# TimD1/vcfdist

Hardware: AMD Instinct MI355X
Metric: supercluster-alignments/sec (higher is better)
Workload: dtype int32; 1 GPU; wgs_synth; superclusters_per_gpu=1000000, span_dist=lognormal(median 20, sigma 1.2) clip [4,10000]

## Files before the change

### include/vcfdist_pr.h

```cpp
#ifndef VCFDIST_PR_H_
#define VCFDIST_PR_H_

#include <stddef.h>
#include <stdint.h>

#ifdef __cplusplus
extern "C" {
#endif

#define VPR_HAPS 4
#define VPR_ALNS 4

#define VPR_PTR_VARIANT 1
#define VPR_PTR_VAR_BEG 2
#define VPR_PTR_VAR_END 4
#define VPR_PTR_INS_LOC 8

#define VPR_TYPE_SUB 1
#define VPR_TYPE_INS 2
#define VPR_TYPE_DEL 3

#define VPR_ERRTYPE_TP 0
#define VPR_ERRTYPE_FP 1
#define VPR_ERRTYPE_FN 2
// ... 50 lines not shown
    const int32_t *sc_end;
    const int64_t *var_off[VPR_HAPS];
    const int32_t *var_pos[VPR_HAPS];
    const uint8_t *var_type[VPR_HAPS];
    const float   *var_qual[VPR_HAPS];
    const int64_t *var_ref_off[VPR_HAPS];
    const int32_t *var_ref_len[VPR_HAPS];
    const int64_t *var_alt_off[VPR_HAPS];
    const int32_t *var_alt_len[VPR_HAPS];
    const uint8_t *allele_pool[VPR_HAPS];
} vpr_variants;

typedef struct vpr_config {
    int32_t device;
    float   max_qual;
    double  credit_threshold;
    double  phase_threshold;
    int64_t workspace_bytes;
    int32_t band_mode;
    int32_t flags;
} vpr_config;
#define VPR_CFG_DENSE_S16 1
#define VPR_CFG_TIE_SMALL_LOGS 2
#define VPR_CFG_GUARD_ALLOC 4
#define VPR_CFG_HAP_DEDUP 16
#define VPR_CFG_KEEP_PATHS 8

typedef struct vpr_results {
    int32_t  *aln_dist;
    uint8_t  *aln_end_plane;
    uint8_t  *aln_beg_plane;
    uint32_t *aln_status;
    int32_t  *sc_phase;
    int32_t  *orig_phase_dist;
    int32_t  *swap_phase_dist;
    uint8_t  *errtype[VPR_HAPS][2];
    int32_t  *sync_group[VPR_HAPS][2];
    float    *credit[VPR_HAPS][2];
    int32_t  *ref_ed[VPR_HAPS][2];
    int32_t  *query_ed[VPR_HAPS][2];
    float    *callq[VPR_HAPS][2];
} vpr_results;

typedef struct vpr_timing {
    double ms_total;
    double ms_prep;
    double ms_fwd;
    double ms_bwd;
    double ms_walk;
    double ms_ed;
    int64_t n_fwd_launches;
    int64_t cells_dense;
    int64_t cells_touched;
    int64_t bytes_algorithmic;
    int64_t n_band_retries;
    int64_t n_tie_replays;
    double  ms_tie;
    double  ms_wall;
    double  ms_wall_phase[6];
    double  ms_host_alloc;
    double  ms_host_blocked;
    int64_t n_alignments_computed;
    int64_t n_device_allocs, n_device_frees, n_host_allocs;
    int64_t n_lane1_seen, n_lane1_finished, n_lane1_waves_dropped;
} vpr_timing;

typedef struct vpr_launch_stat {
    int32_t kind;
    int32_t threads;
    int32_t cells_per_thread;
    int32_t n_units;
    int64_t cells;
    int64_t bytes_algorithmic;
    double  ms;
    int64_t cells_dense;
    char    kernel[32];
} vpr_launch_stat;

typedef struct vpr_handle vpr_handle;

int  vpr_create(const vpr_config *cfg, vpr_handle **out);
void vpr_destroy(vpr_handle *h);
const char *vpr_last_error(const vpr_handle *h);
const char *vpr_version(void);
int vpr_selfcheck_tie_model(int max_entries);

int vpr_run(vpr_handle *h, const vpr_batch *batch, vpr_results *res);
// ... 85 lines not shown
```

### vcfdist_amd/_abi.py

```python
import ctypes as C

import numpy as np

HAPS = 4
ALNS = 4

PTR_VARIANT, PTR_VAR_BEG, PTR_VAR_END, PTR_INS_LOC = 1, 2, 4, 8
TYPE_SUB, TYPE_INS, TYPE_DEL = 1, 2, 3
ERRTYPE_TP, ERRTYPE_FP, ERRTYPE_FN, ERRTYPE_UN = 0, 1, 2, 5
PHASE_ORIG, PHASE_SWAP, PHASE_NONE = 0, 1, 2
PLANE_QUERY, PLANE_REF = 0, 1

ST_SWAP_TIE = 1
ST_WARN_REF_ED = 2
ST_WARN_QUERY_ED = 4
ST_WARN_EXCEEDS = 8
ST_WARN_ZERO_ED = 16
ST_ERR_NO_PTR = 32
ST_ERR_UNFINISHED = 64
ST_ERR_LIMIT = 128
ST_WARN_MASK = ST_WARN_REF_ED | ST_WARN_QUERY_ED | ST_WARN_EXCEEDS | ST_WARN_ZERO_ED

P_i64 = C.POINTER(C.c_int64)
P_i32 = C.POINTER(C.c_int32)
# ... 29 lines not shown
class VprConfig(C.Structure):
    _fields_ = [
        ("device", C.c_int32), ("max_qual", C.c_float),
        ("credit_threshold", C.c_double), ("phase_threshold", C.c_double),
        ("workspace_bytes", C.c_int64), ("band_mode", C.c_int32), ("flags", C.c_int32),
    ]


class VprResults(C.Structure):
    _fields_ = [
        ("aln_dist", P_i32), ("aln_end_plane", P_u8), ("aln_beg_plane", P_u8), ("aln_status", P_u32),
        ("sc_phase", P_i32), ("orig_phase_dist", P_i32), ("swap_phase_dist", P_i32),
        ("errtype", (P_u8 * 2) * HAPS), ("sync_group", (P_i32 * 2) * HAPS),
        ("credit", (P_f32 * 2) * HAPS), ("ref_ed", (P_i32 * 2) * HAPS),
        ("query_ed", (P_i32 * 2) * HAPS), ("callq", (P_f32 * 2) * HAPS),
    ]


CFG_DENSE_S16 = 1
CFG_TIE_SMALL_LOGS = 2
CFG_GUARD_ALLOC = 4
CFG_KEEP_PATHS = 8
CFG_HAP_DEDUP = 16


class VprTiming(C.Structure):
    _fields_ = [
        ("ms_total", C.c_double), ("ms_prep", C.c_double), ("ms_fwd", C.c_double),
        ("ms_bwd", C.c_double), ("ms_walk", C.c_double), ("ms_ed", C.c_double),
        ("n_fwd_launches", C.c_int64), ("cells_dense", C.c_int64), ("cells_touched", C.c_int64),
        ("bytes_algorithmic", C.c_int64), ("n_band_retries", C.c_int64),
        ("n_tie_replays", C.c_int64), ("ms_tie", C.c_double),
        ("ms_wall", C.c_double), ("ms_wall_phase", C.c_double * 6), ("ms_host_alloc", C.c_double),
        ("ms_host_blocked", C.c_double), ("n_alignments_computed", C.c_int64), ("n_device_allocs", C.c_int64), ("n_device_frees", C.c_int64),
        ("n_host_allocs", C.c_int64), ("n_lane1_seen", C.c_int64), ("n_lane1_finished", C.c_int64), ("n_lane1_waves_dropped", C.c_int64),
    ]


class VprLaunchStat(C.Structure):
    _fields_ = [
        ("kind", C.c_int32), ("threads", C.c_int32), ("cells_per_thread", C.c_int32), ("n_units", C.c_int32),
        ("cells", C.c_int64), ("bytes_algorithmic", C.c_int64), ("ms", C.c_double),
        ("cells_dense", C.c_int64), ("kernel", C.c_char * 32),
    ]


class VprSynthParams(C.Structure):
    _fields_ = [
        ("seed", C.c_uint64), ("n_sc", C.c_int32), ("len_mode", C.c_int32),
        ("len_a", C.c_double), ("len_b", C.c_double),
        ("len_min", C.c_int32), ("len_max", C.c_int32),
        ("p_repeat", C.c_double), ("var_per_base", C.c_double), ("p_snp", C.c_double),
        ("indel_mean", C.c_double), ("p_hom", C.c_double), ("p_keep", C.c_double),
        ("p_drop", C.c_double), ("max_qual", C.c_int32), ("reserved", C.c_int32),
        ("p_sv", C.c_double), ("sv_min", C.c_int32), ("sv_max", C.c_int32),
    ]


# ... 375 lines not shown
```

### vcfdist_amd/csrc/pr_api.hip

```cpp
#include <hip/hip_runtime.h>
#include <hip/hip_ext.h>
#include <dlfcn.h>

#include <algorithm>
#include <atomic>
#include <chrono>
#include <cstdarg>
#include <cstdio>
#include <cstdlib>
#include <cstring>
#include <condition_variable>
#include <deque>
#include <functional>
#include <mutex>
#include <string>
#include <thread>
#include <tuple>
#include <unordered_map>
#include <unordered_set>
#include <vector>

#include "../../include/vcfdist_pr.h"
#include "pr_device.h"
#include "pr_plan.h"
// ... 1738 lines not shown
                                  : (its != tie_s.end() ? int64_t(its->second) + 4 + (int64_t(A.y) - A.x) + (int64_t(T.y) - T.x) : int64_t(1) << 30);
                const int64_t lo_all = -(int64_t(d.Lt) - 1);
                int64_t lo0 = lo_all, hi0 = d.Lq - 1, lo1 = lo_all, hi1 = d.Lr - 1;
                if (!tie_full) {
                    lo0 = std::max<int64_t>(lo0, int64_t(A.x) - T.y - M); hi0 = std::min<int64_t>(hi0, int64_t(A.y) - T.x + M);
                    lo1 = std::max<int64_t>(lo1, -int64_t(T.y) - M); hi1 = std::min<int64_t>(hi1, -int64_t(T.x) + M);
                    if (hi0 < lo0) hi0 = lo0;
                    if (hi1 < lo1) hi1 = lo1;
                }
                N.dlo[0] = int32_t(lo0); N.dn[0] = int32_t(hi0 - lo0 + 1);
                N.dlo[1] = int32_t(lo1); N.dn[1] = int32_t(hi1 - lo1 + 1);
            }
            N.cells = int64_t(N.dn[0] + N.dn[1]) * d.Lt + 4;
            if (N.cells >= (int64_t(1) << 32) - 2)
                return fail(h, VPR_ERR_ARG, "supercluster %d alignment %d: (Lq + Lr + 2 Lt) * Lt = %lld stamps exceed the tie replay's 32-bit cell index",
                            d.sc, d.aln, (long long)N.cells);
            N.cap = tie_full ? N.cells : std::min<int64_t>(N.cells, 3 * int64_t(d.Lq + d.Lr + d.Lt) + 4096);
            if (!tie_full && (h->cfg.flags & VPR_CFG_TIE_SMALL_LOGS)) N.cap = 32;
            N.cap = (std::max<int64_t>(2, std::min<int64_t>(N.cap, int64_t(1) << 26)) + 1) & ~int64_t(1);
            int bi = 0;
            while (bi + 1 < TIE_N_BUCKETS && int64_t(TIE_BUCKETS_HOST[bi]) < N.cap) bi++;
            N.bcap = TIE_BUCKETS_HOST[bi];
            N.w_st = (N.cells + 3) & ~int64_t(3); N.w_buf = TIE_BUF_WORDS * N.cap; N.w_bk = (TIE_BKT_WORDS * N.bcap + 8 + 3) & ~int64_t(3);
            const int64_t need = N.w_st + N.w_buf + N.w_bk;
            total += need;
            largest = std::max(largest, need);
            if (early) dec_need += it->second.mode == 2 ? 256 : it->second.n_used;
            needs.push_back(N);
        }
        if (needs.empty()) return VPR_OK;
        trace("    replay: %zu jobs sized", needs.size());
        std::stable_sort(needs.begin(), needs.end(), [](const Need &x, const Need &y) { return x.cells > y.cells; });
        if (tie_job_cur + needs.size() > h->tie_jobs_cap) return fail(h, VPR_ERR_STATE, "tie round: job buffer overflow");
        const bool must = largest * 4 + 256 > scratch_bytes;
        const int64_t room = std::max<int64_t>(h->tie_budget - h->tie_bytes, 0) / 3 * 2;
        const int64_t nb_plan = std::min<int64_t>(std::max<int64_t>(std::min<int64_t>(total * 4, h->tie_scratch_max), 2 * scratch_bytes), room);
        if (must || (total * 4 + 256 > scratch_bytes && scratch_bytes < h->tie_scratch_max && nb_plan > scratch_bytes + scratch_bytes / 2)) {
            const int64_t nb = std::max<int64_t>(nb_plan, largest * 4) + 256;
            void *q = nullptr;
            int64_t got_b = nb;
            h->soft_alloc = !must;
            hipError_t e_sc = x_malloc(h, &q, size_t(nb), SITE);
            h->soft_alloc = false;
            if (e_sc != hipSuccess && must && largest * 4 + 256 < nb) {
                (void)hipGetLastError();
                got_b = largest * 4 + 256;
// ... 21 lines not shown
                int rc_ = dev_alloc(h, &h->d_tie_dec, size_t(nc));
                if (rc_) return rc_;
                h->tie_dec_cap = nc;
                tie_dec_cur = 0;
            }
            dec = h->d_tie_dec + tie_dec_cur;
            n_dec = h->d_tie_ndec + tie_dec_slot;
            tie_patch_slot = tie_dec_slot++; tie_patch_off = tie_dec_cur; tie_patch_cap = dec_cap;
            tie_dec_cur += dec_cap;
        }
        size_t k0 = 0;
        while (k0 < needs.size()) {
            int64_t words = 0;
            size_t k1 = k0;
            TieJob *jobs = h->hp_tie_jobs + tie_job_cur;
            while (k1 < needs.size()) {
                const Need &N = needs[k1];
                const int64_t need = N.w_st + N.w_buf + N.w_bk;
                if (k1 > k0 && (words + need) * 4 > scratch_bytes) break;
                TieJob &J = jobs[k1 - k0];
                memset(&J, 0, sizeof(J));
                J.a = P.work[size_t(off) + N.k];
                J.cap = int32_t(N.cap); J.bcap = int32_t(std::min<int64_t>(N.bcap, 0x7fffffff));
                J.stamp_off = words;
                J.dlo[0] = N.dlo[0]; J.dlo[1] = N.dlo[1]; J.dn[0] = N.dn[0]; J.dn[1] = N.dn[1];
                J.buf_off = words + N.w_st;
                J.bkt_off = (words + N.w_st + N.w_buf) / 2;
                if (early) {
                    const TieEarly &E = tie_early[J.a];
                    const AlnDesc o = plan_desc(h, *E.plan, size_t(E.pos));
                    J.mode = E.mode; J.n_used = E.n_used;
                    J.old_band_w = o.band_w; J.old_pitch[0] = o.pitch[0]; J.old_pitch[1] = o.pitch[1];
                    J.old_mat_off[0] = o.mat_off[0]; J.old_mat_off[1] = o.mat_off[1]; J.old_blo_off = o.blo_off;
                    J.old_arena = E.plan->arena;
                }
                words += need;
                k1++;
            }
            const int32_t nj = int32_t(k1 - k0);
            tie_job_cur += size_t(nj);
            n_tie_jobs += nj;
            if (!tc.tie_first_seen[se]) { tc.tie_first_seen[se] = true; tc.tie_first[se] = words * 4; }
            if (words * 4 > tc.tie_clean[se]) HIPCHK(h, hipMemsetAsync(scratch, 0xff, size_t(words) * 4, ks));
            tc.tie_clean[se] = 0;
            vpr_launch_stat ts_;
            memset(&ts_, 0, sizeof(ts_));
// ... 1058 lines not shown
            for (int iter = 0; na > 0; iter++) {
                HIPCHK(h, hipMemsetAsync(h->d_tie_cnt, 0, 8, st));
                hipLaunchKernelGGL(k_collect_ties, blocks(na), dim3(256), 0, st, h->d_outs, na, h->d_tie_list, h->d_tie_cnt, h->tie_list_cap);
                int32_t n_mark = 0;
                HIPCHK(h, hipMemcpyAsync(&n_mark, h->d_tie_cnt, 4, hipMemcpyDeviceToHost, st));
                HIPCHK(h, hipMemcpyAsync(&n_jobs_pre, h->d_njobs, 4, hipMemcpyDeviceToHost, st));
                HIPCHK(h, x_sync(h, st, SITE));
                n_jobs_final = (n_mark == 0);
                if (n_mark == 0) break;
                if (iter >= 3) return fail(h, VPR_ERR_STATE, "tie pass: %d alignments still marked after %d attempts", n_mark, iter);
                const int32_t n = std::min(n_mark, h->tie_list_cap);
                std::vector<int4> lst;
                lst.resize(size_t(n));
                HIPCHK(h, hipMemcpy(lst.data(), h->d_tie_list, size_t(n) * sizeof(int4), hipMemcpyDeviceToHost));
                if (h->debug) fprintf(stderr, "[vpr] final tie pass %d: %d alignments marked\n", iter, n_mark);
                if ((rc = tie_round(h->lad[2], lst.data(), n, iter > 0, nullptr))) return rc;
                if ((rc = tie_flush(h->lad[2]))) return rc;
                HIPCHK(h, x_sync(h, h->lad[2].ls, SITE));
            }
        }
        return rc;
    }

    void debug_replays() {
        if (h->debug && tie_job_total > 0) {
            std::vector<TieJob> js;
            for (const auto &blk : tie_job_blocks) js.insert(js.end(), blk.first, blk.first + blk.second);
            std::sort(js.begin(), js.end(), [](const TieJob &x, const TieJob &y) { return x.dbg_us > y.dbg_us; });
            int64_t tot_us = 0;
            for (const TieJob &J : js) tot_us += J.dbg_us;
            size_t nf1 = 0, nf2 = 0;
            for (const TieJob &J : js) { nf1 += J.pad == 1; nf2 += J.pad == 2; }
            fprintf(stderr, "[vpr] tie replay: %zu jobs, %.1f ms summed; gave up: %zu (logs), %zu (stamp grid)\n", js.size(), tot_us / 1000.0, nf1, nf2);
            for (const TieJob &J : js)
                if (J.pad == 2 && nf2-- < 4) {
                    const AlnDesc &d = h->descs[size_t(J.a)];
                    fprintf(stderr, "[vpr]   grid too small: sc %d aln %d Lq %d Lr %d Lt %d, diagonals [%d, +%d) [%d, +%d), spans q (%d, %d) t (%d, %d)\n", d.sc, d.aln, d.Lq, d.Lr, d.Lt,
                            J.dlo[0], J.dn[0], J.dlo[1], J.dn[1], h->hp_dspan[d.qs][d.sc].x, h->hp_dspan[d.qs][d.sc].y, h->hp_dspan[d.ts][d.sc].x, h->hp_dspan[d.ts][d.sc].y);
                    fprintf(stderr, "[vpr]     first cell outside: plane %d position %d row %d (wave %d), mode %d\n", J.dbg_oob[0], J.dbg_oob[1], J.dbg_oob[2], J.dbg_oob[3], J.mode);
                }
            for (size_t k = 0; k < js.size() && k < 8; k++) {
                const AlnDesc &d = h->descs[size_t(js[k].a)];
                fprintf(stderr, "[vpr]   sc %d aln %d Lq %d Lr %d Lt %d level %d: %d us, %d waves, %d BFS steps, %d cells; mode %d, consulted %d, decided %d (last in wave %d)\n", d.sc, d.aln,
                        d.Lq, d.Lr, d.Lt, int(h->level[size_t(js[k].a)]), js[k].dbg_us, js[k].dbg_waves, js[k].dbg_steps, js[k].dbg_cells,
                        js[k].mode, js[k].n_used, js[k].dbg_nres, js[k].dbg_lastw);
                fprintf(stderr, "[vpr]     us: BFS %d, patch %d, order A %d B %d suffix %d C %d, seeding %d, setup %d\n", js[k].dbg_t[0], js[k].dbg_t[1],
                        js[k].dbg_t[2], js[k].dbg_t[3], js[k].dbg_t[4], js[k].dbg_t[5], js[k].dbg_t[6], js[k].dbg_t[7]);
                fprintf(stderr, "[vpr]     narrow steps %d: %d not in one row, %d shrinking or growing, %d not reproduced, %d look-ahead steps committing %d levels\n",
                        js[k].dbg_la[0], js[k].dbg_la[1], js[k].dbg_la[2], js[k].dbg_la[3], js[k].dbg_la[4], js[k].dbg_la[5]);
            }
        }
    }

    void debug_levels() {
        if (!h->debug || h->descs.empty()) return;
        std::vector<AlnOut> outs(h->descs.size());
        if (hipMemcpy(outs.data(), h->d_outs, outs.size() * sizeof(AlnOut), hipMemcpyDeviceToHost) != hipSuccess) return;
        static const int32_t edge[6] = {0, 4, 16, 64, 256, 1024};
        for (int lv = 0; lv <= LV_DENSE; lv++) {
            int64_t n[7] = {0, 0, 0, 0, 0, 0, 0};
            double cells[7] = {0, 0, 0, 0, 0, 0, 0};
            for (size_t a = 0; a < outs.size(); a++) {
                if (h->level[a] != lv) continue;
                const AlnDesc &d = h->descs[a];
                int b = 0;
                while (b < 6 && outs[a].s > edge[b]) b++;
                n[b]++;
                cells[b] += double(d.Lq + d.Lr) * d.Lt;
            }
            int64_t tot = 0;
// ... 141 lines not shown
        HIPCHK(h, hipStreamSynchronize(st));
        phase(5);
        lapx("done");
        HIPCHK(h, hipGetLastError());
        (void)need_err_check;
        float ms = 0;
        (void)hipEventElapsedTime(&ms, t0, t1);
        h->timing.ms_total = ms;
        h->timing.ms_fwd = h->timing.ms_bwd = h->timing.ms_walk = h->timing.ms_ed = h->timing.ms_tie = 0;
        for (auto &e : h->events) {
            float m = 0;
            (void)hipEventElapsedTime(&m, e.a, e.b);
            e.st.ms = m;
            if (e.kind == 1) h->timing.ms_fwd += m;
            else if (e.kind == 2) h->timing.ms_bwd += m;
            else if (e.kind == 3) h->timing.ms_walk += m;
            else if (e.kind == 4) h->timing.ms_ed += m;
            else if (e.kind == 6) h->timing.ms_tie += m;
        }
        h->timing.n_fwd_launches = n_fwd;
        h->timing.cells_touched = cells_touched;
        h->timing.n_band_retries = n_retry;
        h->timing.n_tie_replays = n_tie_jobs;
        h->timing.n_alignments_computed = int64_t(h->descs.size()) - h->n_aliased;
        h->timing.n_lane1_seen = h->d_d1_info ? h->hp_tie_cnt[24 + 3] : 0;
        h->timing.n_lane1_finished = h->d_d1_info ? h->hp_tie_cnt[24 + 4] : 0;
        h->timing.n_lane1_waves_dropped = h->d_d1_info ? h->hp_tie_cnt[24 + 1] : 0;
#ifdef D1_CLOCKS
        if (h->debug && h->d_d1_info) {
            int32_t ck[8];
            (void)hipMemcpy(ck, h->d_d1_info + 8, 32, hipMemcpyDeviceToHost);
            fprintf(stderr, "[vpr] k_one_lane passes, longest wave (us): %.1f %.1f %.1f %.1f; pass 1 wave-rows %d of which four slots %d; pass 3 %d / %d\n", ck[0] * 0.01, ck[1] * 0.01,
                    ck[2] * 0.01, ck[3] * 0.01, ck[4], ck[5], ck[6], ck[7]);
        }
#endif
        if (h->debug && h->d_d1_info) fprintf(stderr, "[vpr] distance-1 lane level: %d waves, %d dropped, %d left; %d seen, %d finished (pass 1 %d, pass 2 %d, end cell %d)\n",
                                              h->hp_tie_cnt[24], h->hp_tie_cnt[25], h->hp_tie_cnt[26], h->hp_tie_cnt[27], h->hp_tie_cnt[28], h->hp_tie_cnt[29], h->hp_tie_cnt[30], h->hp_tie_cnt[31]);
        h->timing.ms_wall = phase_ms[5];
        for (int k = 0; k < 6; k++) h->timing.ms_wall_phase[k] = phase_ms[k];
        h->timing.ms_host_alloc = h->hs.ms_alloc;
        h->timing.ms_host_blocked = h->hs.ms_sync;
        h->timing.n_device_allocs = h->hs.n_dev_alloc;
        h->timing.n_device_frees = h->hs.n_dev_free;
        h->timing.n_host_allocs = h->hs.n_pin_alloc;
        if (h->stall_log && phase_ms[5] > stall_dump_ms) {
            std::vector<std::tuple<float, float, const char *, int>> tl;
// ... 56 lines not shown
        phase(0);
        HIPCHK(h, hipEventCreate(&t0));
        HIPCHK(h, hipEventCreate(&t1));
        HIPCHK(h, hipEventRecord(t0, st));
        for (int k = 0; k < 2; k++) {
            LadderCtx &c = h->lad[2 + k];
            c.ls = h->tie_stream[2 * k]; c.ls2 = h->tie_stream[2 * k + 1]; c.ev2 = h->ev_tie2[k];
            c.slot0 = 2 + (2 + k) * LadderCtx::N_SLOTS;
            c.fail_base = (2 + k) * int64_t(h->descs.size()) + int64_t(h->descs.size()) / 16 + 256;
        }
        int rc = VPR_OK;
        h->resident.clear();
        h->res0_cnt = 0;
        if (h->cfg.band_mode == 0) {
            if ((rc = run_dense(h->plan0, h->plan0.d_work, st, false))) return rc;
            if (!h->plan0.chunks.empty()) {
                const Chunk &c = h->plan0.chunks.back();
                h->res0_off = c.work_off; h->res0_cnt = c.count;
            }
        } else if ((rc = round0_windowed())) {
            return rc;
        }
        if ((rc = final_tie_pass())) return rc;
        debug_replays();
        debug_levels();
        lapx("final tie pass done");
        phase(3);
        if ((rc = deferred_edit_distances())) return rc;
        return finish();
    }
};

}

extern "C" {

int vpr_execute(vpr_handle *h) {
    if (!h) return VPR_ERR_ARG;
    if (!h->uploaded) return fail(h, VPR_ERR_STATE, "vpr_execute before vpr_upload");
    dist_free(h);
    for (auto &b : h->exec_blks) b.used = false;
    for (auto &b : h->exec_pins) b.used = false;
    h->hs = vpr_handle::HostStat();
    Exec x(h);
    const int rc = x.run();
    if (x.t0) (void)hipEventDestroy(x.t0);
// ... 9 lines not shown
```

### vcfdist_amd/csrc/pr_tie.hip

```cpp
#ifndef PR_TIE_HIP_
#define PR_TIE_HIP_

#define TIE_NEVER 0xffffffffu
#define TIE_N_BUCKETS 26
#define TIE_BUCKET_LIST {13u, 29u, 59u, 127u, 257u, 541u, 1109u, 2357u, 5087u, 10273u, 20753u, 42043u, 85229u, 172933u, \
                         351061u, 712697u, 1447153u, 2938679u, 5967347u, 12117689u, 24607243u, 49969847u, 101473717u,    \
                         206062531u, 418451333u, 849749479u}
__constant__ uint32_t TIE_BUCKETS[TIE_N_BUCKETS] = TIE_BUCKET_LIST;
static const uint32_t TIE_BUCKETS_HOST[TIE_N_BUCKETS] = TIE_BUCKET_LIST;

struct TieJob {
    int32_t a;
    int32_t cap;
    int32_t bcap;
    int32_t pad;
    int64_t stamp_off;
    int64_t buf_off;
    int64_t bkt_off;
    int32_t mode, n_used;
    int32_t dlo[2], dn[2];
    int32_t old_band_w, old_pitch[2], pad2;
    int64_t old_mat_off[2], old_blo_off;
    uint8_t *old_arena;
    int32_t dbg_us, dbg_steps, dbg_cells, dbg_waves, dbg_nres, dbg_lastw;
    int32_t dbg_oob[4];
    int32_t dbg_la[6];
    int32_t dbg_t[8];
};
#define TIE_BUF_WORDS 10
#define TIE_BLIST 8
#define TIE_BKT_WORDS (2 + 1 + TIE_BLIST)

__device__ __forceinline__ uint32_t tie_ld(const uint32_t *p) {
    return __hip_atomic_load(const_cast<uint32_t *>(p), __ATOMIC_RELAXED, __HIP_MEMORY_SCOPE_AGENT);
}
__device__ __forceinline__ void tie_wait() { asm volatile("s_waitcnt vmcnt(0)" ::: "memory"); }

__device__ __forceinline__ uint8_t *tie_flag_ptr(const AlnDesc &d, uint8_t *ws, const int32_t *blo_all, int p, int x, int t) {
    if (d.band_w == 16) {
        const int2 o = reinterpret_cast<const int2 *>(blo_all + d.blo_off)[t >> 2];
        const int col = x - (p ? o.y : o.x);
        if (col < 0 || col >= 16) return nullptr;
        return ws + d.mat_off[0] + size_t(t >> 2) * 128 + p * 64 + col * 4 + (t & 3);
    }
    if (d.band_w > 0) {
        const int col = x - blo_all[d.blo_off + int64_t(p) * d.Lt + t];
        if (col < 0 || col >= d.band_w) return nullptr;
        return ws + d.mat_off[p] + size_t(t) * d.pitch[p] + col;
    }
    return ws + d.mat_off[p] + size_t(t) * d.pitch[p] + x;
}

#define TIE_U 4
#define TIE_LA 4

template <int TIE_NW>
__global__ void __launch_bounds__(64 * TIE_NW) k_tie_replay(DevBatch B, const AlnDesc *__restrict__ descs,
                                                   TieJob *__restrict__ jobs, int n_jobs, uint8_t *ws,
                                                   const int32_t *__restrict__ blo_all, AlnOut *__restrict__ outs,
                                                   uint32_t *scratch, int32_t *__restrict__ n_overflow,
                                                   int4 *__restrict__ dec, int32_t *__restrict__ n_dec, int dec_cap) {
    constexpr int NT_ = 64 * TIE_NW;
    __shared__ uint32_t mmask[2][1024];
    __shared__ int lds_ntie, lds_nres;
    __shared__ int lds_cnt[3 * TIE_U][TIE_NW];
    __shared__ int lds_or[2][TIE_NW];
    __shared__ int lds_state[2][6];
    __shared__ uint32_t lds_tot[TIE_NW];
    const int j = blockIdx.x;
    if (j >= n_jobs) return;
    __builtin_amdgcn_s_setprio(3);
    const TieJob J = jobs[j];
    const int a = J.a;
    const AlnDesc d = descs[a];
    const int tid = threadIdx.x;
    const int lane = tid & 63, wv = tid >> 6;
    const unsigned long long lt_mask = (1ull << lane) - 1ull;
    int or_par = 0, st_par = 0;
    auto wg_any = [&](bool x) -> bool {
        const bool w_any = __any(x);
        if (lane == 0) lds_or[or_par][wv] = w_any ? 1 : 0;
        __syncthreads();
        bool r = false;
#pragma unroll
        for (int k = 0; k < TIE_NW; k++) r = r || lds_or[or_par][k];
        or_par ^= 1;
        return r;
    };
    const int Lq = d.Lq, Lr = d.Lr, Lt = d.Lt;
    const int s_fin = outs[a].s;
    const unsigned long long clk0 = wall_clock64();
    int dbg_steps = 0, dbg_cells = 0, dbg_waves = 0, dbg_lastw = -1, dbg_nres0 = 0;
    int dbg_la[6] = {0, 0, 0, 0, 0, 0};
    unsigned long long dbg_t[8] = {0, 0, 0, 0, 0, 0, 0, 0}, tk = clk0;
    auto lap = [&](int k) { const unsigned long long now = wall_clock64(); dbg_t[k] += now - tk; tk = now; };
    const uint8_t *seq0 = B.hap_seq[d.qs] + d.q_off, *seq1 = B.ref_seq + d.r_off;
    const int32_t *ptr0 = B.hap_ptr[d.qs] + d.q_off, *ptr1 = B.ref_ptr[d.qs] + d.r_off;
    const uint8_t *flg0 = B.hap_flag[d.qs] + d.q_off, *flg1 = B.ref_flag[d.qs] + d.r_off;
    const uint8_t *Ts = B.hap_seq[d.ts] + d.t_off, *Tf = B.hap_flag[d.ts] + d.t_off;
    const int4 *cand0 = B.cand_q[d.qs] + d.q_off, *cand1 = B.cand_r[d.qs] + d.r_off;
    const int4 *cand20 = B.cand2_q[d.qs] + d.q_off, *cand21 = B.cand2_r[d.qs] + d.r_off;

    uint32_t *stamp = scratch + J.stamp_off;
    uint32_t *buf = scratch + J.buf_off;
    const int cap = J.cap;
    uint2 *qc = reinterpret_cast<uint2 *>(buf), *qn = reinterpret_cast<uint2 *>(buf + 2 * size_t(cap));
    uint32_t *oc = buf + 4 * size_t(cap), *on = buf + 5 * size_t(cap);
    uint32_t *Fa = buf + 6 * size_t(cap), *Ha = buf + 7 * size_t(cap), *Ka = buf + 8 * size_t(cap);
    uint2 *Ta = reinterpret_cast<uint2 *>(buf + 9 * size_t(cap));
    const int tcap = cap / 2;
    unsigned long long *bfirst = reinterpret_cast<unsigned long long *>(scratch) + J.bkt_off;
    uint32_t *bcount = reinterpret_cast<uint32_t *>(bfirst + J.bcap);
    uint32_t *blist = reinterpret_cast<uint32_t *>((reinterpret_cast<uintptr_t>(bcount + J.bcap) + 15) & ~uintptr_t(15));
    const uint32_t sbase1 = uint32_t(J.dn[0]) * uint32_t(Lt);
    const uint32_t s_dummy = sbase1 + uint32_t(J.dn[1]) * uint32_t(Lt);
    bool oob = false;
    int oob_p = 0, oob_q = 0, oob_t = 0;
// ... 318 lines not shown
                    const uint32_t st = tie_ld(stamp + sidx(1 - p, srcs[k], t - 1));
                    if (st == TIE_NEVER || st < wave_lo) continue;
                    nsrc++;
                    if (best < 0 || st > best_st) { best = k; best_st = st; }
                }
                if (best < 0 || (J.mode == 2 && nsrc < 2)) continue;
                if (J.mode) {
                    const int k = atomicAdd(n_dec, 1);
                    if (k < dec_cap) dec[k] = make_int4(a, int(z.x), t, best);
                    atomicAdd(&lds_nres, 1);
                } else {
                    *fp = uint8_t((f & ~uint32_t(F_CHOICE_MASK | F_TIE)) | f_choice_bits(best));
                }
            }
            if (wg_any(oob)) { fail = true; break; }
            if (lds_nres != dbg_nres0) { dbg_nres0 = lds_nres; dbg_lastw = w; }
            if (J.mode == 1 && lds_nres >= J.n_used) { dbg_cells += n_cur; dbg_waves++; break; }
        }
        dbg_cells += n_cur; dbg_waves++;
        lap(1);
        if (w >= s_fin) break;

        const int n = n_cur;
        int done = 0;
        bool have_lam = false;
        while (true) {
            const int room = int(n_bkt) - done;
            const int take = min(room, n - done);
            const int m = done + take;
            tag++;
            const unsigned long long tagw = (unsigned long long)(~tag) << 32;
            for (int b0 = tid; b0 < int(n_bkt); b0 += NT_) bcount[b0] = 0u;
            tie_wait();
            __syncthreads();
            bool blist_full = false;
            for (int i0 = 0; i0 < m; i0 += NT_ * TIE_U) {
                uint32_t e[TIE_U], bk[TIE_U], slot[TIE_U];
                uint2 c[TIE_U];
#pragma unroll
                for (int u = 0; u < TIE_U; u++) {
                    const int i = i0 + u * NT_ + tid;
                    e[u] = (i < m) ? ((have_lam && i < done) ? oc[i] : uint32_t(i)) : 0u;
                }
#pragma unroll
                for (int u = 0; u < TIE_U; u++) c[u] = (i0 + u * NT_ + tid < m) ? qc[e[u]] : make_uint2(0u, 0u);
#pragma unroll
                for (int u = 0; u < TIE_U; u++) {
                    const int i = i0 + u * NT_ + tid;
                    bk[u] = 0u; slot[u] = 0u;
                    if (i >= m) continue;
                    const unsigned long long hv = ((c[u].x >> 31) ? hi_r : hi_q) ^
                                                  ((unsigned long long)(c[u].x & 0x7fffffffu) * 19349669ull + 0xd15f392b3d4704a2ull) ^
                                                  ((unsigned long long)(c[u].y) * 83492791ull);
                    bk[u] = uint32_t(hv % (unsigned long long)n_bkt);
                    Ka[i] = bk[u];
                    Ha[i] = 0u;
                    (void)atomicMin(bfirst + bk[u], tagw | (unsigned long long)uint32_t(i));
                    slot[u] = atomicAdd(bcount + bk[u], 1u);
                }
#pragma unroll
                for (int u = 0; u < TIE_U; u++) {
                    const int i = i0 + u * NT_ + tid;
                    if (i >= m) continue;
                    if (slot[u] < TIE_BLIST) blist[size_t(bk[u]) * TIE_BLIST + slot[u]] = uint32_t(i); else blist_full = true;
                }
            }
            tie_wait();
            blist_full = wg_any(blist_full);
            lap(2);
            for (int i0 = 0; i0 < m; i0 += NT_ * TIE_U) {
                uint32_t b[TIE_U];
                unsigned long long fw[TIE_U];
#pragma unroll
                for (int u = 0; u < TIE_U; u++) b[u] = (i0 + u * NT_ + tid < m) ? Ka[i0 + u * NT_ + tid] : 0u;
#pragma unroll
                for (int u = 0; u < TIE_U; u++)
                    fw[u] = (i0 + u * NT_ + tid < m) ? __hip_atomic_load(bfirst + b[u], __ATOMIC_RELAXED, __HIP_MEMORY_SCOPE_AGENT) : 0ull;
// ... 89 lines not shown
                    const bool act = i < m;
                    const uint32_t f = act ? tie_ld(Fa + i) : 0xffffffffu;
                    const uint32_t e = act ? ((have_lam && i < done) ? oc[i] : uint32_t(i)) : 0u;
                    const uint32_t base = act ? tie_ld(Ka + f) : 0u;
                    const uint32_t g = act ? tie_ld(Ha + f) : 0u;
                    uint32_t intra = 0;
                    for (int l2 = 1; l2 < 64; l2++) {
                        const uint32_t v = uint32_t(__builtin_amdgcn_readlane(int(f), l2));
                        intra += (l2 > lane && v == f) ? 1u : 0u;
                    }
                    if (act) {
                        on[g + base + intra] = e;
                        (void)atomicAdd(Ka + f, 1u);
                    }
                    tie_wait();
                }
            }
            __syncthreads();
            lap(5);
            { uint32_t *tmp = oc; oc = on; on = tmp; }
            have_lam = true;
            done = m;
            if (done == n) break;
            if (bi + 1 >= TIE_N_BUCKETS || TIE_BUCKETS[bi + 1] > uint32_t(J.bcap)) { fail = true; break; }
            n_bkt = TIE_BUCKETS[++bi];
        }
        if (fail) break;

        int n_next = 0;
        wave_lo = cid;
        for (int k0 = 0; k0 < n && !fail; k0 += NT_ * TIE_U) {
            uint32_t e[TIE_U];
            uint2 x[TIE_U];
            bool t0[TIE_U], t1[TIE_U], t2[TIE_U];
            uint32_t j0[TIE_U], j1[TIE_U], j2[TIE_U];
#pragma unroll
            for (int u = 0; u < TIE_U; u++) e[u] = (k0 + u * NT_ + tid < n) ? oc[k0 + u * NT_ + tid] : 0u;
#pragma unroll
            for (int u = 0; u < TIE_U; u++) x[u] = (k0 + u * NT_ + tid < n) ? qc[e[u]] : make_uint2(0u, 0u);
#pragma unroll
            for (int u = 0; u < TIE_U; u++) {
                const bool act = k0 + u * NT_ + tid < n;
                const int p = int(x[u].x >> 31), q = int(x[u].x & 0x7fffffffu), t = int(x[u].y);
                t0[u] = act && q + 1 < (p ? Lr : Lq); t1[u] = act && t + 1 < Lt; t2[u] = t0[u] && t1[u];
                const uint32_t c0 = cid + 3u * uint32_t(u * NT_ + tid);
                j0[u] = t0[u] ? sidx(p, q + 1, t) : 0u; j1[u] = t1[u] ? sidx(p, q, t + 1) : 0u; j2[u] = t2[u] ? sidx(p, q + 1, t + 1) : 0u;
                if (t0[u]) (void)atomicMin(stamp + j0[u], c0);
                if (t1[u]) (void)atomicMin(stamp + j1[u], c0 + 1u);
                if (t2[u]) (void)atomicMin(stamp + j2[u], c0 + 2u);
            }
            tie_wait();
            __syncthreads();
            bool w0[TIE_U], w1[TIE_U], w2[TIE_U];
#pragma unroll
            for (int u = 0; u < TIE_U; u++) {
                const uint32_t c0 = cid + 3u * uint32_t(u * NT_ + tid);
                w0[u] = t0[u] && tie_ld(stamp + j0[u]) == c0;
                w1[u] = t1[u] && tie_ld(stamp + j1[u]) == c0 + 1u;
                w2[u] = t2[u] && tie_ld(stamp + j2[u]) == c0 + 2u;
            }
            unsigned long long b0_[TIE_U], b1_[TIE_U], b2_[TIE_U];
#pragma unroll
// ... 22 lines not shown
                n_next += tot;
            }
            cid += 3u * uint32_t(min(NT_ * TIE_U, n - k0));
            if (cid > 0xf0000000u || any_oob_) fail = true;
            tie_wait();
            __syncthreads();
        }
        if (fail) break;
        lap(6);
        { uint2 *tmp = qc; qc = qn; qn = tmp; }
        n_cur = n_next;
        if (n_cur == 0) { fail = true; break; }
    }
    if (fail && tid == 0) atomicAdd(n_overflow, 1);
    const bool any_oob = wg_any(oob);
    if (oob && lane == int(__builtin_ctzll(__ballot(oob)))) { jobs[j].dbg_oob[0] = oob_p; jobs[j].dbg_oob[1] = oob_q; jobs[j].dbg_oob[2] = oob_t; jobs[j].dbg_oob[3] = dbg_waves; }
    if (tid == 0) jobs[j].pad = fail ? (any_oob ? 2 : 1) : 0;
    if (tid == 0) {
        jobs[j].dbg_us = int32_t((wall_clock64() - clk0) / 100);
        jobs[j].dbg_steps = dbg_steps; jobs[j].dbg_cells = dbg_cells; jobs[j].dbg_waves = dbg_waves;
        jobs[j].dbg_nres = lds_nres; jobs[j].dbg_lastw = dbg_lastw;
        for (int k = 0; k < 8; k++) jobs[j].dbg_t[k] = int32_t(dbg_t[k] / 100);
        for (int k = 0; k < 6; k++) jobs[j].dbg_la[k] = dbg_la[k];
    }
}

__global__ void k_tie_patch(const AlnDesc *__restrict__ descs, const int4 *__restrict__ dec, const int32_t *__restrict__ n_dec,
                            int dec_cap, uint8_t *ws, int tag) {
    const int i = blockIdx.x * blockDim.x + threadIdx.x;
    if (i >= min(*n_dec, dec_cap)) return;
    const int4 e = dec[i];
    const AlnDesc d = descs[e.x];
    if (d.band_pad != tag) return;
    uint8_t *fp = tie_flag_ptr(d, ws, reinterpret_cast<const int32_t *>(ws), int(uint32_t(e.y) >> 31), e.y & 0x7fffffff, e.z);
    if (!fp) return;
    const uint32_t f = *fp;
    if (!(f & F_SWP)) return;
    *fp = uint8_t((f & ~uint32_t(F_CHOICE_MASK | F_TIE)) | f_choice_bits(e.w));
}

#endif
```

Baseline: 196.6 million supercluster-alignments/s.

## Order small tie-replay frontiers in LDS instead of global bucket tables

Adds an LDS-resident path for the tie-replay frontier ordering. Frontiers of up to 64 cells are ordered with wave-level readlane ranking, and frontiers of up to 512 cells go through a shared-memory hash table with a counting sort. This avoids the global bucket-table clears and atomics, and skips allocating bucket workspace for small jobs. It also raises the launch-bounds occupancy hint and adds ordering counters. The cost is more shared memory per block, which may lower occupancy, plus extra branching. The old global path stays available behind a config flag.

```diff
diff --git a/include/vcfdist_pr.h b/include/vcfdist_pr.h
--- a/include/vcfdist_pr.h
+++ b/include/vcfdist_pr.h
@@ -96,6 +96,7 @@
 } vpr_config;
 #define VPR_CFG_DENSE_S16 1
 #define VPR_CFG_TIE_SMALL_LOGS 2
+#define VPR_CFG_TIE_GLOBAL_ORDER 32
 #define VPR_CFG_GUARD_ALLOC 4
 #define VPR_CFG_HAP_DEDUP 16
 #define VPR_CFG_KEEP_PATHS 8
@@ -137,6 +138,11 @@
     int64_t n_alignments_computed;
     int64_t n_device_allocs, n_device_frees, n_host_allocs;
     int64_t n_lane1_seen, n_lane1_finished, n_lane1_waves_dropped;
+    int64_t n_tie_order_wave, n_tie_order_lds, n_tie_order_global;
+    int64_t n_tie_order_lds_rehash;
+    int64_t n_tie_order_handover;
+    int64_t n_tie_order_big_bucket;
+    int64_t n_tie_jobs_mode[3];
 } vpr_timing;
 
 typedef struct vpr_launch_stat {
diff --git a/vcfdist_amd/_abi.py b/vcfdist_amd/_abi.py
--- a/vcfdist_amd/_abi.py
+++ b/vcfdist_amd/_abi.py
@@ -75,6 +75,7 @@
 CFG_GUARD_ALLOC = 4
 CFG_KEEP_PATHS = 8
 CFG_HAP_DEDUP = 16
+CFG_TIE_GLOBAL_ORDER = 32
 
 
 class VprTiming(C.Structure):
@@ -87,6 +88,9 @@
         ("ms_wall", C.c_double), ("ms_wall_phase", C.c_double * 6), ("ms_host_alloc", C.c_double),
         ("ms_host_blocked", C.c_double), ("n_alignments_computed", C.c_int64), ("n_device_allocs", C.c_int64), ("n_device_frees", C.c_int64),
         ("n_host_allocs", C.c_int64), ("n_lane1_seen", C.c_int64), ("n_lane1_finished", C.c_int64), ("n_lane1_waves_dropped", C.c_int64),
+        ("n_tie_order_wave", C.c_int64), ("n_tie_order_lds", C.c_int64), ("n_tie_order_global", C.c_int64),
+        ("n_tie_order_lds_rehash", C.c_int64), ("n_tie_order_handover", C.c_int64), ("n_tie_order_big_bucket", C.c_int64),
+        ("n_tie_jobs_mode", C.c_int64 * 3),
     ]
 
 
diff --git a/vcfdist_amd/csrc/pr_api.hip b/vcfdist_amd/csrc/pr_api.hip
--- a/vcfdist_amd/csrc/pr_api.hip
+++ b/vcfdist_amd/csrc/pr_api.hip
@@ -1784,6 +1784,7 @@
             while (bi + 1 < TIE_N_BUCKETS && int64_t(TIE_BUCKETS_HOST[bi]) < N.cap) bi++;
             N.bcap = TIE_BUCKETS_HOST[bi];
             N.w_st = (N.cells + 3) & ~int64_t(3); N.w_buf = TIE_BUF_WORDS * N.cap; N.w_bk = (TIE_BKT_WORDS * N.bcap + 8 + 3) & ~int64_t(3);
+            if (N.cap <= TIE_LDS_N && !(h->cfg.flags & VPR_CFG_TIE_GLOBAL_ORDER)) { N.bcap = 0; N.w_bk = 0; }
             const int64_t need = N.w_st + N.w_buf + N.w_bk;
             total += need;
             largest = std::max(largest, need);
@@ -1851,6 +1852,7 @@
                 memset(&J, 0, sizeof(J));
                 J.a = P.work[size_t(off) + N.k];
                 J.cap = int32_t(N.cap); J.bcap = int32_t(std::min<int64_t>(N.bcap, 0x7fffffff));
+                J.no_lds = (h->cfg.flags & VPR_CFG_TIE_GLOBAL_ORDER) ? 1 : 0;
                 J.stamp_off = words;
                 J.dlo[0] = N.dlo[0]; J.dlo[1] = N.dlo[1]; J.dn[0] = N.dn[0]; J.dn[1] = N.dn[1];
                 J.buf_off = words + N.w_st;
@@ -2955,6 +2957,15 @@
         return rc;
     }
 
+    int64_t n_tie_order[7] = {0, 0, 0, 0, 0, 0, 0}, n_tie_mode[3] = {0, 0, 0};
+    void count_orders() {
+        for (const auto &blk : tie_job_blocks)
+            for (size_t k = 0; k < blk.second; k++) {
+                for (int q = 0; q < 7; q++) n_tie_order[q] += blk.first[k].n_order[q];
+                n_tie_mode[std::min(std::max(blk.first[k].mode, 0), 2)]++;
+            }
+    }
+
     void debug_replays() {
         if (h->debug && tie_job_total > 0) {
             std::vector<TieJob> js;
@@ -2965,6 +2976,21 @@
             size_t nf1 = 0, nf2 = 0;
             for (const TieJob &J : js) { nf1 += J.pad == 1; nf2 += J.pad == 2; }
             fprintf(stderr, "[vpr] tie replay: %zu jobs, %.1f ms summed; gave up: %zu (logs), %zu (stamp grid)\n", js.size(), tot_us / 1000.0, nf1, nf2);
+            {
+                int64_t t[8] = {0, 0, 0, 0, 0, 0, 0, 0}, tl[2] = {0, 0}, hist[12] = {0, 0, 0, 0, 0, 0, 0, 0, 0, 0, 0, 0}, no[4] = {0, 0, 0, 0}, waves = 0, cells = 0, steps = 0;
+                for (const TieJob &J : js) {
+                    for (int k = 0; k < 8; k++) t[k] += J.dbg_t[k];
+                    for (int k = 0; k < 12; k++) hist[k] += J.dbg_hist[k];
+                    for (int k = 0; k < 4; k++) no[k] += J.n_order[k];
+                    waves += J.dbg_waves; cells += J.dbg_cells; steps += J.dbg_steps;
+                    tl[0] += J.dbg_t_lds[0]; tl[1] += J.dbg_t_lds[1];
+                }
+                fprintf(stderr, "[vpr] tie passes: jobs %zu us %lld slowest_us %d waves %lld cells %lld bfs_steps %lld | us bfs %lld patch %lld order_a %lld order_b %lld suffix %lld order_c %lld seeding %lld setup %lld order_wave %lld order_lds %lld | order_n_hist",
+                        js.size(), (long long)tot_us, js.empty() ? 0 : js[0].dbg_us, (long long)waves, (long long)cells, (long long)steps, (long long)t[0], (long long)t[1], (long long)t[2],
+                        (long long)t[3], (long long)t[4], (long long)t[5], (long long)t[6], (long long)t[7], (long long)tl[0], (long long)tl[1]);
+                for (int k = 0; k < 12; k++) fprintf(stderr, " %lld", (long long)hist[k]);
+                fprintf(stderr, " | order_iters wave %lld lds %lld global %lld rehash %lld\n", (long long)no[0], (long long)no[1], (long long)no[2], (long long)no[3]);
+            }
             for (const TieJob &J : js)
                 if (J.pad == 2 && nf2-- < 4) {
                     const AlnDesc &d = h->descs[size_t(J.a)];
@@ -2977,8 +3003,8 @@
                 fprintf(stderr, "[vpr]   sc %d aln %d Lq %d Lr %d Lt %d level %d: %d us, %d waves, %d BFS steps, %d cells; mode %d, consulted %d, decided %d (last in wave %d)\n", d.sc, d.aln,
                         d.Lq, d.Lr, d.Lt, int(h->level[size_t(js[k].a)]), js[k].dbg_us, js[k].dbg_waves, js[k].dbg_steps, js[k].dbg_cells,
                         js[k].mode, js[k].n_used, js[k].dbg_nres, js[k].dbg_lastw);
-                fprintf(stderr, "[vpr]     us: BFS %d, patch %d, order A %d B %d suffix %d C %d, seeding %d, setup %d\n", js[k].dbg_t[0], js[k].dbg_t[1],
-                        js[k].dbg_t[2], js[k].dbg_t[3], js[k].dbg_t[4], js[k].dbg_t[5], js[k].dbg_t[6], js[k].dbg_t[7]);
+                fprintf(stderr, "[vpr]     us: BFS %d, patch %d, order A %d B %d suffix %d C %d (LDS paths: %d, %d), seeding %d, setup %d\n", js[k].dbg_t[0], js[k].dbg_t[1],
+                        js[k].dbg_t[2], js[k].dbg_t[3], js[k].dbg_t[4], js[k].dbg_t[5], js[k].dbg_t_lds[0], js[k].dbg_t_lds[1], js[k].dbg_t[6], js[k].dbg_t[7]);
                 fprintf(stderr, "[vpr]     narrow steps %d: %d not in one row, %d shrinking or growing, %d not reproduced, %d look-ahead steps committing %d levels\n",
                         js[k].dbg_la[0], js[k].dbg_la[1], js[k].dbg_la[2], js[k].dbg_la[3], js[k].dbg_la[4], js[k].dbg_la[5]);
             }
@@ -3166,6 +3192,9 @@
         h->timing.cells_touched = cells_touched;
         h->timing.n_band_retries = n_retry;
         h->timing.n_tie_replays = n_tie_jobs;
+        h->timing.n_tie_order_wave = n_tie_order[0]; h->timing.n_tie_order_lds = n_tie_order[1]; h->timing.n_tie_order_global = n_tie_order[2];
+        h->timing.n_tie_order_lds_rehash = n_tie_order[4]; h->timing.n_tie_order_handover = n_tie_order[5]; h->timing.n_tie_order_big_bucket = n_tie_order[6];
+        for (int k = 0; k < 3; k++) h->timing.n_tie_jobs_mode[k] = n_tie_mode[k];
         h->timing.n_alignments_computed = int64_t(h->descs.size()) - h->n_aliased;
         h->timing.n_lane1_seen = h->d_d1_info ? h->hp_tie_cnt[24 + 3] : 0;
         h->timing.n_lane1_finished = h->d_d1_info ? h->hp_tie_cnt[24 + 4] : 0;
@@ -3268,6 +3297,7 @@
             return rc;
         }
         if ((rc = final_tie_pass())) return rc;
+        count_orders();
         debug_replays();
         debug_levels();
         lapx("final tie pass done");
diff --git a/vcfdist_amd/csrc/pr_tie.hip b/vcfdist_amd/csrc/pr_tie.hip
--- a/vcfdist_amd/csrc/pr_tie.hip
+++ b/vcfdist_amd/csrc/pr_tie.hip
@@ -19,17 +19,24 @@
     int64_t bkt_off;
     int32_t mode, n_used;
     int32_t dlo[2], dn[2];
-    int32_t old_band_w, old_pitch[2], pad2;
+    int32_t old_band_w, old_pitch[2];
+    int32_t no_lds;
     int64_t old_mat_off[2], old_blo_off;
     uint8_t *old_arena;
     int32_t dbg_us, dbg_steps, dbg_cells, dbg_waves, dbg_nres, dbg_lastw;
     int32_t dbg_oob[4];
     int32_t dbg_la[6];
     int32_t dbg_t[8];
+    int32_t dbg_hist[12];
+    int32_t n_order[7], pad3;
+    int32_t dbg_t_lds[2];
 };
 #define TIE_BUF_WORDS 10
 #define TIE_BLIST 8
 #define TIE_BKT_WORDS (2 + 1 + TIE_BLIST)
+#define TIE_LDS_N 512
+#define TIE_LDS_T (2 * TIE_LDS_N)
+#define TIE_LDS_MAX_BKT ((1u << 23) - 1u)
 
 __device__ __forceinline__ uint32_t tie_ld(const uint32_t *p) {
     return __hip_atomic_load(const_cast<uint32_t *>(p), __ATOMIC_RELAXED, __HIP_MEMORY_SCOPE_AGENT);
@@ -55,7 +62,7 @@
 #define TIE_LA 4
 
 template <int TIE_NW>
-__global__ void __launch_bounds__(64 * TIE_NW) k_tie_replay(DevBatch B, const AlnDesc *__restrict__ descs,
+__global__ void __launch_bounds__(64 * TIE_NW, 2) k_tie_replay(DevBatch B, const AlnDesc *__restrict__ descs,
                                                    TieJob *__restrict__ jobs, int n_jobs, uint8_t *ws,
                                                    const int32_t *__restrict__ blo_all, AlnOut *__restrict__ outs,
                                                    uint32_t *scratch, int32_t *__restrict__ n_overflow,
@@ -67,6 +74,10 @@
     __shared__ int lds_or[2][TIE_NW];
     __shared__ int lds_state[2][6];
     __shared__ uint32_t lds_tot[TIE_NW];
+    __shared__ uint32_t ord_tab[TIE_LDS_T];
+    __shared__ uint16_t ord_lam[TIE_LDS_N];
+    __shared__ uint2 ord_qc[TIE_LDS_N];
+    static_assert(TIE_LDS_N % NT_ == 0 || NT_ % TIE_LDS_N == 0, "elements per thread");
     const int j = blockIdx.x;
     if (j >= n_jobs) return;
     __builtin_amdgcn_s_setprio(3);
@@ -92,7 +103,8 @@
     const unsigned long long clk0 = wall_clock64();
     int dbg_steps = 0, dbg_cells = 0, dbg_waves = 0, dbg_lastw = -1, dbg_nres0 = 0;
     int dbg_la[6] = {0, 0, 0, 0, 0, 0};
-    unsigned long long dbg_t[8] = {0, 0, 0, 0, 0, 0, 0, 0}, tk = clk0;
+    int dbg_hist[12] = {0, 0, 0, 0, 0, 0, 0, 0, 0, 0, 0, 0}, n_order[7] = {0, 0, 0, 0, 0, 0, 0};
+    unsigned long long dbg_t[10] = {0, 0, 0, 0, 0, 0, 0, 0, 0, 0}, tk = clk0;
     auto lap = [&](int k) { const unsigned long long now = wall_clock64(); dbg_t[k] += now - tk; tk = now; };
     const uint8_t *seq0 = B.hap_seq[d.qs] + d.q_off, *seq1 = B.ref_seq + d.r_off;
     const int32_t *ptr0 = B.hap_ptr[d.qs] + d.q_off, *ptr1 = B.ref_ptr[d.qs] + d.r_off;
@@ -457,12 +469,147 @@
         if (w >= s_fin) break;
 
         const int n = n_cur;
+        dbg_hist[n <= 1 ? 0 : min(11, 32 - __clz(n - 1))]++;
         int done = 0;
         bool have_lam = false;
+        bool lam_lds = false;
+        auto bucket_of = [&](const uint2 c) -> uint32_t {
+            const unsigned long long hv = ((c.x >> 31) ? hi_r : hi_q) ^
+                                          ((unsigned long long)(c.x & 0x7fffffffu) * 19349669ull + 0xd15f392b3d4704a2ull) ^
+                                          ((unsigned long long)(c.y) * 83492791ull);
+            return uint32_t(hv % (unsigned long long)n_bkt);
+        };
         while (true) {
             const int room = int(n_bkt) - done;
             const int take = min(room, n - done);
             const int m = done + take;
+            if (done) n_order[3]++;
+            if (!J.no_lds && m <= TIE_LDS_N && n_bkt <= TIE_LDS_MAX_BKT && (!have_lam || lam_lds)) {
+                if (done) n_order[4]++;
+                if (m <= 64) {
+                    n_order[0]++;
+                    if (wv == 0) {
+                        const bool act = lane < m;
+                        const uint32_t e = act ? ((have_lam && lane < done) ? uint32_t(ord_lam[lane]) : uint32_t(lane)) : 0u;
+                        const uint2 c = act ? qc[e] : make_uint2(0u, 0u);
+                        const uint32_t bk = act ? bucket_of(c) : 0xffffffffu;
+                        int first = lane;
+                        for (int l = m - 1; l >= 0; l--) first = (uint32_t(__builtin_amdgcn_readlane(int(bk), l)) == bk) ? l : first;
+                        const int key = first * 64 + lane;
+                        int pos = 0, same = 0;
+                        for (int l = 0; l < m; l++) { const int kl = __builtin_amdgcn_readlane(key, l); pos += (kl > key) ? 1 : 0; same += ((kl >> 6) == first) ? 1 : 0; }
+                        if (__any(act && same > TIE_BLIST)) n_order[6]++;
+                        if (act) { ord_lam[pos] = uint16_t(e); ord_qc[pos] = c; }
+                    }
+                    __syncthreads();
+                    lap(8);
+                } else {
+                    n_order[1]++;
+                    constexpr int PER = (TIE_LDS_N + NT_ - 1) / NT_;
+                    uint32_t *hc = ord_tab;
+                    uint16_t *g16 = reinterpret_cast<uint16_t *>(ord_tab + TIE_LDS_N), *tmp16 = g16 + TIE_LDS_N;
+                    uint32_t e[PER], bk[PER], sl[PER], f[PER];
+                    uint2 c[PER];
+                    for (int s0 = tid; s0 < TIE_LDS_T; s0 += NT_) ord_tab[s0] = 0xffffffffu;
+#pragma unroll
+                    for (int u = 0; u < PER; u++) {
+                        const int i = tid + u * NT_;
+                        e[u] = (i < m) ? ((have_lam && i < done) ? uint32_t(ord_lam[i]) : uint32_t(i)) : 0u;
+                    }
+#pragma unroll
+                    for (int u = 0; u < PER; u++) c[u] = (tid + u * NT_ < m) ? qc[e[u]] : make_uint2(0u, 0u);
+#pragma unroll
+                    for (int u = 0; u < PER; u++) bk[u] = (tid + u * NT_ < m) ? bucket_of(c[u]) : 0u;
+                    __syncthreads();
+#pragma unroll
+                    for (int u = 0; u < PER; u++) {
+                        const int i = tid + u * NT_;
+                        sl[u] = 0u;
+                        if (i >= m) continue;
+                        const uint32_t pk = (bk[u] << 9) | uint32_t(i);
+                        uint32_t s_ = (bk[u] * 2654435761u) >> 22;
+                        static_assert(TIE_LDS_T == 1024 && TIE_LDS_N == 512, "slot and index bits");
+                        while (true) {
+                            uint32_t cur = ord_tab[s_];
+                            if (cur == 0xffffffffu) {
+                                cur = atomicCAS(ord_tab + s_, 0xffffffffu, pk);
+                                if (cur == 0xffffffffu) break;
+                            }
+                            if ((cur >> 9) == bk[u]) { (void)atomicMin(ord_tab + s_, pk); break; }
+                            s_ = (s_ + 1u) & uint32_t(TIE_LDS_T - 1);
+                        }
+                        sl[u] = s_;
+                    }
+                    __syncthreads();
+#pragma unroll
+                    for (int u = 0; u < PER; u++) f[u] = ord_tab[sl[u]] & 511u;
+                    __syncthreads();
+                    for (int s0 = tid; s0 < TIE_LDS_N; s0 += NT_) hc[s0] = 0u;
+                    __syncthreads();
+#pragma unroll
+                    for (int u = 0; u < PER; u++) if (tid + u * NT_ < m) (void)atomicAdd(hc + f[u], 1u);
+                    __syncthreads();
+                    {
+                        uint32_t h_[PER], tsum = 0;
+#pragma unroll
+                        for (int u = 0; u < PER; u++) { const int f_ = tid * PER + u; h_[u] = (f_ < m) ? (hc[f_] & 0xffffu) : 0u; tsum += h_[u]; }
+                        uint32_t suf = tsum;
+#pragma unroll
+                        for (int o = 1; o < 64; o <<= 1) {
+                            const uint32_t tv = uint32_t(__shfl_down(int(suf), o));
+                            if (lane + o < 64) suf += tv;
+                        }
+                        if (lane == 0) lds_tot[wv] = suf;
+                        __syncthreads();
+                        uint32_t acc = suf - tsum;
+#pragma unroll
+                        for (int k = 0; k < TIE_NW; k++) acc += (k > wv) ? lds_tot[k] : 0u;
+#pragma unroll
+                        for (int u = PER - 1; u >= 0; u--) { const int f_ = tid * PER + u; if (f_ < TIE_LDS_N) g16[f_] = uint16_t(acc); acc += h_[u]; }
+                    }
+                    __syncthreads();
+                    uint32_t g[PER];
+#pragma unroll
+                    for (int u = 0; u < PER; u++) {
+                        const int i = tid + u * NT_;
+                        g[u] = 0u;
+                        if (i >= m) continue;
+                        g[u] = g16[f[u]];
+                        const uint32_t k_ = atomicAdd(hc + f[u], 0x10000u) >> 16;
+                        tmp16[g[u] + k_] = uint16_t(i);
+                    }
+                    __syncthreads();
+                    bool big = false;
+#pragma unroll
+                    for (int u = 0; u < PER; u++) {
+                        const int i = tid + u * NT_;
+                        if (i >= m) continue;
+                        const uint32_t cn = hc[f[u]] & 0xffffu;
+                        big = big || cn > TIE_BLIST;
+                        uint32_t rank = 0;
+                        for (uint32_t k_ = 0; k_ < cn; k_++) rank += (uint32_t(tmp16[g[u] + k_]) > uint32_t(i)) ? 1u : 0u;
+                        ord_lam[g[u] + rank] = uint16_t(e[u]);
+                        ord_qc[g[u] + rank] = c[u];
+                    }
+                    if (wg_any(big)) n_order[6]++;
+                    lap(9);
+                }
+                have_lam = true; lam_lds = true;
+                done = m;
+                if (done == n) break;
+                if (bi + 1 >= TIE_N_BUCKETS) { fail = true; break; }
+                n_bkt = TIE_BUCKETS[++bi];
+                continue;
+            }
+            if (n_bkt > uint32_t(J.bcap)) { fail = true; break; }
+            if (have_lam && lam_lds) {
+                n_order[5]++;
+                for (int i0 = tid; i0 < done; i0 += NT_) oc[i0] = uint32_t(ord_lam[i0]);
+                tie_wait();
+                __syncthreads();
+                lam_lds = false;
+            }
+            n_order[2]++;
             tag++;
             const unsigned long long tagw = (unsigned long long)(~tag) << 32;
             for (int b0 = tid; b0 < int(n_bkt); b0 += NT_) bcount[b0] = 0u;
@@ -484,10 +631,7 @@
                     const int i = i0 + u * NT_ + tid;
                     bk[u] = 0u; slot[u] = 0u;
                     if (i >= m) continue;
-                    const unsigned long long hv = ((c[u].x >> 31) ? hi_r : hi_q) ^
-                                                  ((unsigned long long)(c[u].x & 0x7fffffffu) * 19349669ull + 0xd15f392b3d4704a2ull) ^
-                                                  ((unsigned long long)(c[u].y) * 83492791ull);
-                    bk[u] = uint32_t(hv % (unsigned long long)n_bkt);
+                    bk[u] = bucket_of(c[u]);
                     Ka[i] = bk[u];
                     Ha[i] = 0u;
                     (void)atomicMin(bfirst + bk[u], tagw | (unsigned long long)uint32_t(i));
@@ -623,10 +767,11 @@
             have_lam = true;
             done = m;
             if (done == n) break;
-            if (bi + 1 >= TIE_N_BUCKETS || TIE_BUCKETS[bi + 1] > uint32_t(J.bcap)) { fail = true; break; }
+            if (bi + 1 >= TIE_N_BUCKETS) { fail = true; break; }
             n_bkt = TIE_BUCKETS[++bi];
         }
         if (fail) break;
+        const bool seed_lds = lam_lds;
 
         int n_next = 0;
         wave_lo = cid;
@@ -636,9 +781,13 @@
             bool t0[TIE_U], t1[TIE_U], t2[TIE_U];
             uint32_t j0[TIE_U], j1[TIE_U], j2[TIE_U];
 #pragma unroll
-            for (int u = 0; u < TIE_U; u++) e[u] = (k0 + u * NT_ + tid < n) ? oc[k0 + u * NT_ + tid] : 0u;
-#pragma unroll
-            for (int u = 0; u < TIE_U; u++) x[u] = (k0 + u * NT_ + tid < n) ? qc[e[u]] : make_uint2(0u, 0u);
+            for (int u = 0; u < TIE_U; u++) e[u] = (!seed_lds && k0 + u * NT_ + tid < n) ? oc[k0 + u * NT_ + tid] : 0u;
+#pragma unroll
+            for (int u = 0; u < TIE_U; u++) {
+                const int k = k0 + u * NT_ + tid;
+                x[u] = make_uint2(0u, 0u);
+                if (k < n) x[u] = seed_lds ? ord_qc[k] : qc[e[u]];
+            }
 #pragma unroll
             for (int u = 0; u < TIE_U; u++) {
                 const bool act = k0 + u * NT_ + tid < n;
@@ -707,6 +856,9 @@
         jobs[j].dbg_nres = lds_nres; jobs[j].dbg_lastw = dbg_lastw;
         for (int k = 0; k < 8; k++) jobs[j].dbg_t[k] = int32_t(dbg_t[k] / 100);
         for (int k = 0; k < 6; k++) jobs[j].dbg_la[k] = dbg_la[k];
+        for (int k = 0; k < 12; k++) jobs[j].dbg_hist[k] = dbg_hist[k];
+        for (int k = 0; k < 7; k++) jobs[j].n_order[k] = n_order[k];
+        for (int k = 0; k < 2; k++) jobs[j].dbg_t_lds[k] = int32_t(dbg_t[8 + k] / 100);
     }
 }
 
```

Result: no change. 196.3 million supercluster-alignments/s, median of 4 (-0.1%).
